# sriramelango/optimized-diffusion-model

Hardware: AMD Instinct MI355X
Metric: trajectories/sec (1000-step PC sampler, NCSN++ [1,9,9], bs=128/GPU) (higher is better)
Workload: dtype f32; 1 GPU; NCSN++ nf=64 ch_mult=[1,2,2] on [128,1,9,9] per GPU, 1000-step reflected PC sampler (predictor euler_maruyama, corrector none), classifier-free guidance on (2B-sample forwards), fp32; global_batch=128, num_scales=1000, score_evals_per_traj=999, parallelism=single GPU

## Files before the change

### optimized-diffusion-model_amd/csrc/common.h

```cpp
#pragma once
#include <hip/hip_runtime.h>

typedef float f32x4 __attribute__((vector_size(16)));

extern __shared__ __attribute__((aligned(16))) unsigned char rdmi_lds[];

#define RDMI_THREADS 256

#if defined(__HIP_DEVICE_COMPILE__)
#define RDMI_SCHED_FENCE() __builtin_amdgcn_sched_barrier(0)
#else
#define RDMI_SCHED_FENCE() ((void)0)
#endif

__device__ __forceinline__ float silu_f(float y) { return __fdividef(y, 1.0f + __expf(-y)); }

__device__ __forceinline__ f32x4 mfma16(float a, float b, f32x4 c) {
    return __builtin_amdgcn_mfma_f32_16x16x4f32(a, b, c, 0, 0, 0);
}

__device__ __forceinline__ f32x4 mfma4(float a, float b, f32x4 c) {
    return __builtin_amdgcn_mfma_f32_4x4x1f32(a, b, c, 0, 0, 0);
}

typedef unsigned short bf16_t;
typedef unsigned int u32x4 __attribute__((vector_size(16)));
#if defined(__HIP_DEVICE_COMPILE__)
typedef __bf16 rdmi_bf16x8 __attribute__((ext_vector_type(8)));
__device__ __forceinline__ bf16_t f2bf(float f) { return __builtin_bit_cast(unsigned short, (__bf16)f); }
__device__ __forceinline__ f32x4 mfma16_bf16(u32x4 a, u32x4 b, f32x4 c) {
    return __builtin_amdgcn_mfma_f32_16x16x32_bf16(__builtin_bit_cast(rdmi_bf16x8, a), __builtin_bit_cast(rdmi_bf16x8, b), c, 0, 0, 0);
}
#else
__device__ __forceinline__ bf16_t f2bf(float f) {
    unsigned u = __builtin_bit_cast(unsigned, f);
    if ((u & 0x7fffffffu) > 0x7f800000u) return (bf16_t)((u >> 16) | 0x40);
    return (bf16_t)((u + 0x7fffu + ((u >> 16) & 1u)) >> 16);
}
#if defined(RDMI_EMU)
__device__ __forceinline__ float bf2f_host(bf16_t h) { const unsigned u = (unsigned)h << 16; return __builtin_bit_cast(float, u); }
__device__ __forceinline__ f32x4 mfma16_bf16(u32x4 a, u32x4 b, f32x4 c) {
    bf16_t A[64][8], B[64][8];
    std::memcpy(A, emu::wave_exchange(&a, 16), sizeof A);
    std::memcpy(B, emu::wave_exchange(&b, 16), sizeof B);
    const int lane = emu::lane_id(), col = lane & 15;
    for (int e = 0; e < 4; ++e) {
        const int r = (lane >> 4) * 4 + e;
        float s = c[e];
        for (int k = 0; k < 32; ++k) s += bf2f_host(A[r + 16 * (k >> 3)][k & 7]) * bf2f_host(B[col + 16 * (k >> 3)][k & 7]);
        c[e] = s;
    }
    return c;
}
#else
__device__ __forceinline__ f32x4 mfma16_bf16(u32x4, u32x4, f32x4 c) { abort(); return c; }
#endif
#endif
#if defined(__HIP_DEVICE_COMPILE__)
__device__ __forceinline__ void wave_order_point() { __builtin_amdgcn_wave_barrier(); }
#elif defined(RDMI_EMU)
__device__ __forceinline__ void wave_order_point() { int z = 0; (void)emu::wave_exchange(&z, sizeof z); }
#else
__device__ __forceinline__ void wave_order_point() {}
#endif
#if defined(__HIP_DEVICE_COMPILE__)
// ... 12 lines not shown
#elif defined(RDMI_EMU)
__device__ __forceinline__ void glds16(const void* g, unsigned wave_off) { std::memcpy(rdmi_lds + wave_off + 16 * emu::lane_id(), g, 16); }
#else
__device__ __forceinline__ void glds16(const void*, unsigned) {}
#endif
#if defined(__HIP_DEVICE_COMPILE__)
__device__ __forceinline__ int mad_u24(int a, int b, int c) { return (int)(__umul24((unsigned)a, (unsigned)b) + (unsigned)c); }
#else
__device__ __forceinline__ int mad_u24(int a, int b, int c) { return a * b + c; }
#endif
__device__ __forceinline__ unsigned pack_bf16x2(float lo, float hi) { return (unsigned)f2bf(lo) | ((unsigned)f2bf(hi) << 16); }
__device__ __forceinline__ float bf2f(bf16_t h) { return __builtin_bit_cast(float, (unsigned)h << 16); }
__device__ __forceinline__ f32x4 ldact4(const float* base, size_t idx, int bf) {
    if (bf) {
        typedef unsigned int u32x2 __attribute__((vector_size(8)));
        const u32x2 u = *reinterpret_cast<const u32x2*>(reinterpret_cast<const bf16_t*>(base) + idx);
        return f32x4{__builtin_bit_cast(float, u[0] << 16), __builtin_bit_cast(float, u[0] & 0xffff0000u), __builtin_bit_cast(float, u[1] << 16),
                     __builtin_bit_cast(float, u[1] & 0xffff0000u)};
    }
    return *reinterpret_cast<const f32x4*>(base + idx);
}
__device__ __forceinline__ float ldact1(const float* base, size_t idx, int bf) { return bf ? bf2f(reinterpret_cast<const bf16_t*>(base)[idx]) : base[idx]; }
__device__ __forceinline__ void stact1(float* base, size_t idx, float v, int bf) {
    if (bf) reinterpret_cast<bf16_t*>(base)[idx] = f2bf(v); else base[idx] = v;
}

#if defined(__HIP_DEVICE_COMPILE__)
template <int CTRL>
__device__ __forceinline__ float dpp_f(float v) {
    return __builtin_bit_cast(float, __builtin_amdgcn_update_dpp(0, __builtin_bit_cast(int, v), CTRL, 0xf, 0xf, true));
}
__device__ __forceinline__ float row16_sum(float v) {
    v += dpp_f<0xB1>(v); v += dpp_f<0x4E>(v); v += dpp_f<0x141>(v); v += dpp_f<0x140>(v);
    return v;
}
__device__ __forceinline__ float row16_max(float v) {
    v = fmaxf(v, dpp_f<0xB1>(v)); v = fmaxf(v, dpp_f<0x4E>(v)); v = fmaxf(v, dpp_f<0x141>(v)); v = fmaxf(v, dpp_f<0x140>(v));
    return v;
}
__device__ __forceinline__ float row8_sum(float v) {
    v += dpp_f<0xB1>(v); v += dpp_f<0x4E>(v); v += dpp_f<0x141>(v);
    return v;
}
__device__ __forceinline__ float lane_bcast(float v, int l) { return __builtin_bit_cast(float, __builtin_amdgcn_readlane(__builtin_bit_cast(int, v), l)); }
#else
__device__ __forceinline__ float row16_sum(float v) { v += __shfl_xor(v, 1); v += __shfl_xor(v, 2); v += __shfl_xor(v, 4); v += __shfl_xor(v, 8); return v; }
__device__ __forceinline__ float row16_max(float v) {
    v = fmaxf(v, __shfl_xor(v, 1)); v = fmaxf(v, __shfl_xor(v, 2)); v = fmaxf(v, __shfl_xor(v, 4)); v = fmaxf(v, __shfl_xor(v, 8));
    return v;
}
__device__ __forceinline__ float row8_sum(float v) { v += __shfl_xor(v, 1); v += __shfl_xor(v, 2); v += __shfl_xor(v, 4); return v; }
__device__ __forceinline__ float lane_bcast(float v, int l) { return __shfl(v, l); }
#endif
__device__ __forceinline__ float group32_sum(float v, int lane) {
    const float r = row16_sum(v);
    const float s0 = lane_bcast(r, 0), s1 = lane_bcast(r, 16), s2 = lane_bcast(r, 32), s3 = lane_bcast(r, 48);
    return lane < 32 ? s0 + s1 : s2 + s3;
}
__device__ __forceinline__ float group64_sum(float v) {
    const float r = row16_sum(v);
    return (lane_bcast(r, 0) + lane_bcast(r, 16)) + (lane_bcast(r, 32) + lane_bcast(r, 48));
}

__device__ __forceinline__ float reflect_f(float x) {
    float m = x - 2.0f * floorf(x * 0.5f);
    m = (m >= 2.0f) ? 0.0f : m;
    return (m > 1.0f) ? 2.0f - m : m;
}

__device__ __forceinline__ f32x4 ldg4(const float* p) {
#if defined(__HIP_DEVICE_COMPILE__)
    typedef const f32x4 __attribute__((address_space(1))) * gptr_t;
    return *(gptr_t)(p);
#else
    return *reinterpret_cast<const f32x4*>(p);
#endif
}
__device__ __forceinline__ float ldg1(const float* p) {
#if defined(__HIP_DEVICE_COMPILE__)
    typedef const float __attribute__((address_space(1))) * gptr_t;
    return *(gptr_t)(p);
#else
    return *p;
#endif
}

__device__ __forceinline__ void stg1(float* p, float v) {
#if defined(__HIP_DEVICE_COMPILE__)
    typedef float __attribute__((address_space(1))) * gptr_t;
    *(gptr_t)(p) = v;
#else
    *p = v;
#endif
}
__device__ __forceinline__ void stg4(float* p, f32x4 v) {
#if defined(__HIP_DEVICE_COMPILE__)
    typedef f32x4 __attribute__((address_space(1))) * gptr_t;
    *(gptr_t)(p) = v;
#else
    *reinterpret_cast<f32x4*>(p) = v;
#endif
}

#if defined(__HIP_DEVICE_COMPILE__)
typedef unsigned int xq_t __attribute__((ext_vector_type(4)));
struct XBuf { __amdgpu_buffer_rsrc_t r; };
// ... 60 lines not shown
```

### optimized-diffusion-model_amd/csrc/rdmi.hip

```cpp
#include <hip/hip_runtime.h>

#include <algorithm>
#include <cmath>
#include <cstdarg>
#include <cstdio>
#include <cstdlib>
#include <cstring>
#include <climits>
#include <map>
#include <memory>
#include <stdexcept>
#include <string>
#include <vector>

#include "../../include/rdmi.h"
#include "attn_kernel.h"
#include "conv_kernel.h"
#include "misc_kernels.h"
#include "unet_kernel.h"
#include "bwd_kernels.h"
#include "opt_kernels.h"
#include "ode_kernels.h"
#include "tiled_kernels.h"

// ... 1337 lines not shown
        o.main_ph.lds_off = in.off; o.main_ph.rs = in.rs; o.main_ph.nch = in.C / 16;
        for (int t = 0; t < 4; ++t) o.tab_off[t] = up4_table(in.H, in.W, t);
        o.w_tile_stride = 4 * in.C * o.Cout_pad * (int)sizeof(float);
        o.dst_off = dst->off; o.dst_rs = dst->rs;
        if (o.main_ph.nch % 8 != 0 || o.rows <= 4 || o.dst_kind != 0 || in.C != Cout || in.hw() != 16 || in.pm || cur_samp < 0 || dst->C != Cout || dst->hw() != o.rows)
            fail_("folded upsample conv: unsupported shape (" + std::to_string(in.H) + "x" + std::to_string(in.W) + " source, " + std::to_string(in.C) + " -> " + std::to_string(Cout) + " channels)");
        dst->pm = true;
        const int idx = emit(o);
        patch_arena(idx, F_W, c->wmap.at(wkey + ".up4"));
        patch_param(idx, F_BIAS, bias_param);
        return idx;
    }
};

FusedBuilder::LT fused_resblock(FusedBuilder& b, const std::string& name, FusedBuilder::LT& xin, int cout, int dense_off) {
    using LT = FusedBuilder::LT;
    const int H = xin.H, W = xin.W;
    const float rs2 = (float)(1.0 / std::sqrt(2.0));
    if (xin.C != cout) {
        LT out = b.talloc(cout, H, W);
        b.conv(xin, H, W, H, W, 1, 0, 1, name + ".NIN_0", 0, cout, name + ".NIN_0.b", 0, 0, &out, 1.f, -1, nullptr, nullptr, "", "");
        b.gn(xin, name + ".GroupNorm_0", true);
        LT h1 = b.talloc(cout, H, W);
        b.conv(xin, H, W, H, W, 1, 1, 9, name + ".Conv_0", 0, cout, name + ".Conv_0.bias", 0, 0, &h1, 1.f, dense_off, nullptr, nullptr, "", "");
        b.tfree(xin);
        b.gn(h1, name + ".GroupNorm_1", true);
        b.conv(h1, H, W, H, W, 1, 1, 9, name + ".Conv_1", 0, cout, name + ".Conv_1.bias", 0, 0, &out, rs2, -1, &out, nullptr, "", "");
        b.tfree(h1);
        return out;
    }
    LT xact = b.talloc(xin.C, H, W);
    b.gn(xact, name + ".GroupNorm_0", true, &xin);
    LT h1 = b.talloc(cout, H, W);
    b.conv(xact, H, W, H, W, 1, 1, 9, name + ".Conv_0", 0, cout, name + ".Conv_0.bias", 0, 0, &h1, 1.f, dense_off, nullptr, nullptr, "", "");
    b.tfree(xact);
    b.gn(h1, name + ".GroupNorm_1", true);
    LT out = b.talloc(cout, H, W);
    b.conv(h1, H, W, H, W, 1, 1, 9, name + ".Conv_1", 0, cout, name + ".Conv_1.bias", 0, 0, &out, rs2, -1, &xin, nullptr, "", "");
    b.tfree(h1);
    b.tfree(xin);
    return out;
}

FusedBuilder::LT fused_attn(FusedBuilder& b, const std::string& name, FusedBuilder::LT& x) {
    using LT = FusedBuilder::LT;
    rdmi_ctx* c = b.c;
    const int C = x.C, H = x.H, W = x.W, L = H * W, Lpad = pad16(L);
    if (C != 64 || Lpad > 96) { b.fail_("attention: only C=64, H*W<=96 is built"); return x; }
    if (b.cur_samp < 0) { b.fail_("attention inside the multi-sample (low-resolution) section is not built"); return x; }
    LT xn = b.talloc(C, H, W);
    b.gn(xn, name + ".GroupNorm_0", false, &x);
    LT q = b.talloc(C, H, W), k = b.talloc(C, H, W);
    const int ps = Lpad + 4;
    const int vt_bytes = C * ps * 4, p_bytes = L * ps * 4;
    const int vt_off = b.alloc_top(vt_bytes);
    const bool fold3 = !b.train && std::getenv("RDMI_NO_ATTN_FOLD") == nullptr;
    const size_t bq = c->wmap.at(name + (fold3 ? ".bqkvf" : ".bqkv"));
    {
        const int idx = b.conv(xn, H, W, H, W, 1, 0, 1, name + (fold3 ? ".qkv3f" : ".qkv3"), 0, 3 * C, "", bq, 3, &q, 1.f, -1, nullptr, nullptr, "", "");
        FOp& o = b.prog.fprog[(size_t)idx];
        o.dst2_off = k.off; o.dst3_off = vt_off; o.dst3_rs = ps; o.split_C = C;
        o.qkv1 = (std::getenv("RDMI_NO_QKV1") == nullptr && o.ntap == 1 && o.main_ph.nch == 4 && o.Cout_pad == 192 && C == 64 && o.mtiles <= 6) ? 1 : 0;
    }
    b.tfree(xn);
    const int p_off = b.alloc_top(p_bytes);
    LT o = b.talloc(C, H, W);
    {
        FOp a = b.blank(FOP_ATTN);
        a.q_off = q.off; a.k_off = k.off; a.qk_rs = q.rs; a.vt_off = vt_off; a.p_off = p_off; a.ps = ps;
        a.L = L; a.Lpad = Lpad; a.C = C; a.att_scale = 1.0f / std::sqrt((float)C);
        a.dst_off = o.off; a.dst_rs = o.rs;
        if (fold3) { a.resid_off = x.off; a.resid_rs = x.rs; a.scale = (float)(1.0 / std::sqrt(2.0)); }
        const int ia = b.emit(a);
        if (fold3) b.patch_param(ia, FusedBuilder::F_BIAS, name + ".NIN_3.b");
    }
    b.tfree(q); b.tfree(k);
    b.free_bytes(vt_off, vt_bytes); b.free_bytes(p_off, p_bytes);
    if (fold3) { b.tfree(x); return o; }
    LT out = b.talloc(C, H, W);
    b.conv(o, H, W, H, W, 1, 0, 1, name + ".NIN_3", 0, C, name + ".NIN_3.b", 0, 0, &out, (float)(1.0 / std::sqrt(2.0)), -1, &x, nullptr, "", "");
    b.tfree(o);
    b.tfree(x);
    return out;
}

int build_fused_program_pass(rdmi_ctx* c, rdmi_ctx::FusedProg& q, int S, int TAB_RESERVE, int TAB1_RESERVE, int* tab_used, int* tab1_used, bool coop, bool train);

int build_one_program(rdmi_ctx* c, int S, bool coop = false, bool train = false) {
    int used = 0, used1 = 0;
    {
        rdmi_ctx::FusedProg sizing;
        if (int e = build_fused_program_pass(c, sizing, S, 8 * 1024, 24 * 1024, &used, &used1, coop, train)) return e;
    }
    rdmi_ctx::FusedProg q;
    if (int e = build_fused_program_pass(c, q, S, (used + 63) & ~63, (used1 + 63) & ~63, &used, &used1, coop, train)) return e;
    c->progs.push_back(std::move(q));
    return 0;
}

int resident_workgroups() {
#ifdef RDMI_EMU
    return 256;
#else
    int dev = 0, cus = 0;
    if (hipGetDevice(&dev) != hipSuccess || hipDeviceGetAttribute(&cus, hipDeviceAttributeMultiprocessorCount, dev) != hipSuccess) return 0;
    return cus;
#endif
// ... 1317 lines not shown
```

### optimized-diffusion-model_amd/csrc/unet_kernel.h

```cpp
#pragma once
#include <cstddef>

#include "common.h"

#define UW_THREADS 512
#define UW_WAVES 8
#ifndef UW_PF_M4
#define UW_PF_M4 4
#endif
#ifndef UW_PF_N1
#define UW_PF_N1 4
#endif
#ifndef UW_PF_KS1
#define UW_PF_KS1 4
#endif
#ifndef UW_PRIO
#define UW_PRIO 0
#endif
#ifndef UW_LIGHT_BARRIER
#define UW_LIGHT_BARRIER 0
#endif

__device__ __forceinline__ void lds_barrier() {
#if defined(__HIP_DEVICE_COMPILE__) && UW_LIGHT_BARRIER
// ... 735 lines not shown
    const int col = nt * 16 + lrow;
    const int gcol = min(col, o_Cout - 1) >> 2, G4 = o_Cout >> 2;
    const float* slots = lds_f(OPI(w, gn_slot_off));
    const float inv_cnt = OPF(w, inv_cnt), eps = OPF(w, eps);
    const int act = OPI(w, gn_act), rs = OPI(w, gn_rs);
    float* dstp = lds_f(OPI(w, gn_off));
    float mean = 0.f, rstd = 0.f;
    if (o_samp >= 0) {
        const float* slot = slots + (size_t)gcol * nslots * 2;
        float s1 = 0.f, s2 = 0.f;
        for (int k = 0; k < nslots; k += 2) {
            const f32x4 p = *reinterpret_cast<const f32x4*>(slot + 2 * k);
            s1 += p[0]; s2 += p[1]; s1 += p[2]; s2 += p[3];
        }
        mean = s1 * inv_cnt;
        rstd = (1.0f / sqrtf(fmaxf(s2 * inv_cnt - mean * mean, 0.f) + eps)) * gmul;
    }
#pragma unroll
    for (int i = 0; i < 4; ++i)
        if (i < nmt) {
            if (o_samp < 0) {
                float s1, s2;
                if (hw_shift == 4) {
                    const float* slot = slots + (size_t)((mt0 + i * WM) * G4 + gcol) * 8;
                    const f32x4 p = *reinterpret_cast<const f32x4*>(slot), q = *reinterpret_cast<const f32x4*>(slot + 4);
                    s1 = (p[0] + p[2]) + (q[0] + q[2]); s2 = (p[1] + p[3]) + (q[1] + q[3]);
                } else { s1 = ps1[i]; s2 = ps2[i]; }
                mean = s1 * inv_cnt;
                rstd = (1.0f / sqrtf(fmaxf(s2 * inv_cnt - mean * mean, 0.f) + eps)) * gmul;
            }
            const int row0 = (mt0 + i * WM) * 16 + kq * 4;
#pragma unroll
            for (int r = 0; r < 4; ++r) {
                const float y = (acc[i][r] - mean) * rstd + gadd;
                float ya = act ? silu_f(y) : y;
                if (TR) {
                    const int dop = OPI(w, drop_op);
                    if (dop >= 0 && u.drop_p > 0.f)
                        ya *= dropout_scale((uint64_t)*u.seed_dev, (uint32_t)dop, ((uint64_t)min(n0, u.NB - 1) * o_rows + (row0 + r)) * o_Cout + col, u.drop_p);
                }
                if (row0 + r < o_rows && col < o_Cout) dstp[(row0 + r) * rs + col] = ya;
            }
        }
}

__device__ __forceinline__ void fconv_qkv(const OpW& w, const UnetArgs& u, int wave, int lane) {
    const int lrow = lane & 15, kq = lane >> 4;
    const int wn = wave & 3, wm = wave >> 2;
    const int o_rows = OPI(w, rows), mtiles = OPI(w, mtiles), o_Cout_pad = OPI(w, Cout_pad);
    const int m_lds = OPI(w, main_ph.lds_off), m_rs = OPI(w, main_ph.rs);
    const float* m_w = OPP(w, const float, main_ph.w);
    const float* o_bias = OPP(w, const float, bias);
    const float o_scale = OPF(w, scale);
    const int sc_ = OPI(w, split_C), o_dst = OPI(w, dst_off), o_dst2 = OPI(w, dst2_off), o_dst3 = OPI(w, dst3_off), o_dst_rs = OPI(w, dst_rs), rs3 = OPI(w, dst3_rs);
    const short* tab = reinterpret_cast<const short*>(rdmi_lds + opw_at(w, (int)(offsetof(FOp, tab_off) / 4)));
    const size_t bstride = (size_t)o_Cout_pad * 16;
    f32x4 bf[3][4];
    float add[3];
#pragma unroll
    for (int c = 0; c < 3; ++c) {
        const int col = (wn + 4 * c) * 16 + lrow;
        add[c] = ldg1(o_bias + col);
#pragma unroll
        for (int ch = 0; ch < 4; ++ch) bf[c][ch] = ldg4(m_w + (size_t)col * 16 + kq * 4 + (size_t)ch * bstride);
    }
    int abase[3];
#pragma unroll
    for (int i = 0; i < 3; ++i) abase[i] = arow(tab, min((wm + 2 * i) * 16 + lrow, mtiles * 16 - 1), m_lds, m_rs, u.zero_off) + kq * 16;
    f32x4 acc[3][3];
#pragma unroll
    for (int i = 0; i < 3; ++i)
#pragma unroll
        for (int c = 0; c < 3; ++c) acc[i][c] = f32x4{0.f, 0.f, 0.f, 0.f};
#pragma unroll
    for (int ch = 0; ch < 4; ++ch) {
        f32x4 af[3];
#pragma unroll
        for (int i = 0; i < 3; ++i) af[i] = *reinterpret_cast<const f32x4*>(rdmi_lds + abase[i] + ch * 64);
#pragma unroll
        for (int j = 0; j < 4; ++j)
#pragma unroll
            for (int i = 0; i < 3; ++i)
#pragma unroll
                for (int c = 0; c < 3; ++c) acc[i][c] = mfma16(af[i][j], bf[c][ch][j], acc[i][c]);
    }
    const int lc = wn * 16 + lrow;
    (void)sc_;
#pragma unroll
    for (int i = 0; i < 3; ++i) {
        const int mt = wm + 2 * i;
        if (mt >= mtiles) continue;
        const int row0 = mt * 16 + kq * 4;
#pragma unroll
        for (int c = 0; c < 2; ++c) {
            float* dstp = lds_f(c == 0 ? o_dst : o_dst2);
#pragma unroll
            for (int r = 0; r < 4; ++r)
                if (row0 + r < o_rows) dstp[(row0 + r) * o_dst_rs + lc] = (acc[i][c][r] + add[c]) * o_scale;
        }
        f32x4 v = acc[i][2];
        for (int r = 0; r < 4; ++r) v[r] = (v[r] + add[2]) * o_scale;
        *reinterpret_cast<f32x4*>(lds_f(o_dst3) + lc * rs3 + row0) = v;
    }
}

template <bool DIAG, bool MS, bool TR = false>
__device__ __forceinline__ void fop_conv(const OpW& w, const UnetArgs& u, int n0, int wave, int lane, long long* fine) {
    const int ntiles = OPI(w, Cout_pad) >> 4, mtiles = OPI(w, mtiles);
    const int lWN = (ntiles >= 8 && (ntiles & 7) == 0) ? 3 : (ntiles >= 4 ? 2 : (ntiles >= 2 ? 1 : 0));
    const int WN = 1 << lWN, WM = UW_WAVES >> lWN, lWM = 3 - lWN;
    const int wn = wave & (WN - 1), wm = wave >> lWN;
    const int o_Cout = OPI(w, Cout), o_dense = OPI(w, dense_off);
    const float* o_bias = OPP(w, const float, bias); const float* o_bias2 = OPP(w, const float, bias2);
    if (OPI(w, dst_kind) == 3 && OPI(w, qkv1)) { fconv_qkv(w, u, wave, lane); return; }
    const bool fused_gn = OPI(w, dst_kind) == 0 && OPI(w, gn_off) >= 0;
    const int wts = OPI(w, w_tile_stride);
    const int o_samp = MS ? OPI(w, samp) : 0, hw_shift = MS ? OPI(w, hw_shift) : 0;
    const float* dense_base = u.dense + (size_t)max(o_dense, 0);
    f32x4 acc[4];
    float ps1[4] = {0.f, 0.f, 0.f, 0.f}, ps2[4] = {0.f, 0.f, 0.f, 0.f};
    const int wcol = min(wn * 16 + (lane & 15), o_Cout - 1);
    float gmul = ldg1((fused_gn ? OPP(w, const float, gamma) : o_bias) + wcol), gadd = ldg1((fused_gn ? OPP(w, const float, beta) : o_bias) + wcol);
    int k_mt0 = 0, k_nt = 0, k_nmt = 0;
    for (int nt = wn; nt < ntiles; nt += WN) {
        const int col = nt * 16 + (lane & 15), colc = min(col, o_Cout - 1);
        float add1 = ldg1(o_bias + colc), add2 = ldg1((o_bias2 ? o_bias2 : o_bias) + colc);
        for (int mt0 = wm; mt0 < mtiles; mt0 += wts ? WM : 4 * WM) {
            const int left = (mtiles - mt0 + WM - 1) >> lWM;
            const int nmt = wts ? 1 : (left >= 4 ? 4 : left);
            float daddm[4] = {0.f, 0.f, 0.f, 0.f};
            float dv = ldg1(dense_base + (o_dense >= 0 ? (size_t)min(n0 + max(o_samp, 0), u.NB - 1) * u.dense_stride + colc : 0));
            if (MS && o_dense >= 0 && o_samp < 0) {
#pragma unroll
                for (int i = 0; i < 4; ++i)
                    if (i < nmt) {
                        const int sl = ((mt0 + i * WM) * 16 + (lane >> 4) * 4) >> hw_shift;
                        daddm[i] = ldg1(dense_base + (size_t)min(n0 + sl, u.NB - 1) * u.dense_stride + colc);
                    }
            }
            const bool tapm = (OPI(w, main_ph.nch) & 3) == 0;
            const bool tapm8 = (OPI(w, main_ph.nch) & 7) == 0;
            switch (nmt) {
                case 1:
                    if (OPI(w, rows) <= 4 && OPI(w, dst_kind) != 1 && OPI(w, dst_kind) != 3) {
                        if (tapm8) fconv_main_t<DIAG, 1, false, 8, true>(w, u, mt0, WM, nt, lane, fine, acc);
                        else fconv_main<DIAG, 1, UW_PF_M4, true>(w, u, mt0, WM, nt, lane, fine, acc);
                    } else if (tapm8) fconv_main_t<DIAG, 1, false, 8>(w, u, mt0, WM, nt, lane, fine, acc, (unsigned)mt0 * (unsigned)wts);
                    else if (tapm) fconv_main_t<DIAG, 1>(w, u, mt0, WM, nt, lane, fine, acc);
                    else fconv_main<DIAG, 1, UW_PF_N1>(w, u, mt0, WM, nt, lane, fine, acc);
                    break;
                case 2: fconv_main<DIAG, 2, 8>(w, u, mt0, WM, nt, lane, fine, acc); break;
                case 3: {
                    const int last_rows = OPI(w, rows) - (mt0 + 2 * WM) * 16;
                    const bool lm4 = last_rows >= 1 && last_rows <= 4 && OPI(w, dst_kind) != 1 && OPI(w, dst_kind) != 3;
                    if (tapm) { if (lm4) fconv_main_t<DIAG, 3, true>(w, u, mt0, WM, nt, lane, fine, acc); else fconv_main_t<DIAG, 3>(w, u, mt0, WM, nt, lane, fine, acc); }
// ... 114 lines not shown
#pragma unroll
    for (int k = 0; k < KMAX; ++k) {
        const int p = tid + k * UW_THREADS;
        if (p < np && !withhold) {
            f32x2 v;
            if (mode == 0) v = *reinterpret_cast<const f32x2*>(lds_f(0) + at(p, m));
            else {
                const int i = p << 1, row = i >> csh, c = i & (Cs - 1);
                v = *reinterpret_cast<const f32x2*>(lds_f(a_off) + row * a_rs + c);
                *reinterpret_cast<f32x2*>(lds_f(0) + at(p, m)) = v;
            }
            const float v0 = v[0], v1 = v[1];
            xbuf_store16(xb, gbase + (unsigned)m * slotb + (unsigned)p * 16u, __builtin_bit_cast(unsigned, v0), __builtin_bit_cast(unsigned, v1), epoch);
        }
    }
    const int nk = (np + UW_THREADS - 1) / UW_THREADS;
    u32x4 y[3 * KMAX];
    unsigned long long spins = 0;
    bool broken = __hip_atomic_load(u.coop_err, __ATOMIC_RELAXED, __HIP_MEMORY_SCOPE_AGENT) != 0;
    if (broken) *failw = 1;
    for (; !broken;) {
#pragma unroll
        for (int k = 0; k < KMAX; ++k)
            if (k < nk) {
                const unsigned po = (unsigned)min(tid + k * UW_THREADS, np - 1) * 16u;
#pragma unroll
                for (int jj = 0; jj < 3; ++jj) y[k * 3 + jj] = xbuf_load16(xb, gbase + (unsigned)((m + 1 + jj) & 3) * slotb + po);
            }
        bool ok = true;
#pragma unroll
        for (int k = 0; k < KMAX; ++k)
            if (k < nk) {
#pragma unroll
                for (int jj = 0; jj < 3; ++jj) { const unsigned t1 = y[k * 3 + jj][1], t3 = y[k * 3 + jj][3]; ok &= t1 == epoch && t3 == epoch; }
            }
        if (ok) break;
        if (++spins > RDMI_SPIN_LIMIT) { *failw = 1; __hip_atomic_store(u.coop_err, 1, __ATOMIC_RELAXED, __HIP_MEMORY_SCOPE_AGENT); break; }
        spin_relax();
    }
#pragma unroll
    for (int k = 0; k < KMAX; ++k) {
        const int p = tid + k * UW_THREADS;
        if (!broken && k < nk && p < np) {
#pragma unroll
            for (int jj = 0; jj < 3; ++jj) {
                const unsigned a = y[k * 3 + jj][0], b = y[k * 3 + jj][2];
                *reinterpret_cast<f32x2*>(lds_f(0) + at(p, (m + 1 + jj) & 3)) = f32x2{__builtin_bit_cast(float, a), __builtin_bit_cast(float, b)};
            }
        }
    }
}

__device__ __forceinline__ void fop_attn(const OpW& w, int wave, int lane) {
    struct { int L, Lpad, q_off, k_off, vt_off, p_off, qk_rs, ps, C, dst_off, dst_rs; float att_scale; } o;
    o.L = OPI(w, L); o.Lpad = OPI(w, Lpad); o.q_off = OPI(w, q_off); o.k_off = OPI(w, k_off); o.vt_off = OPI(w, vt_off); o.p_off = OPI(w, p_off);
    o.qk_rs = OPI(w, qk_rs); o.ps = OPI(w, ps); o.C = OPI(w, C); o.dst_off = OPI(w, dst_off); o.dst_rs = OPI(w, dst_rs); o.att_scale = OPF(w, att_scale);
    const int lrow = lane & 15, kq = lane >> 4;
    const int L = o.L, mtiles = o.Lpad >> 4;
    const float* Q = lds_f(o.q_off);
    const float* K = lds_f(o.k_off);
    const float* Vt = lds_f(o.vt_off);
    float* P = lds_f(o.p_off);
    const int rs = o.qk_rs, ps = o.ps;
    const int nchq = o.C >> 4;
    for (int mt = wave; mt < mtiles; mt += UW_WAVES) {
        f32x4 s[6];
#pragma unroll
        for (int t = 0; t < 6; ++t) s[t] = f32x4{0.f, 0.f, 0.f, 0.f};
        const int qrow = min(mt * 16 + lrow, L - 1);
        for (int ch = 0; ch < nchq; ++ch) {
            const f32x4 af = *reinterpret_cast<const f32x4*>(Q + (size_t)qrow * rs + ch * 16 + kq * 4);
#pragma unroll
            for (int t = 0; t < 6; ++t) {
                if (t < mtiles) {
                    const int krow = min(t * 16 + lrow, L - 1);
                    const f32x4 bf = *reinterpret_cast<const f32x4*>(K + (size_t)krow * rs + ch * 16 + kq * 4);
#pragma unroll
                    for (int j = 0; j < 4; ++j) s[t] = mfma16(af[j], bf[j], s[t]);
                }
            }
        }
#pragma unroll
        for (int r = 0; r < 4; ++r) {
            float mx = -3.0e38f;
#pragma unroll
            for (int t = 0; t < 6; ++t)
                if (t < mtiles && t * 16 + lrow < L) { s[t][r] *= o.att_scale; mx = fmaxf(mx, s[t][r]); }
            mx = row16_max(mx);
            float sum = 0.f;
#pragma unroll
            for (int t = 0; t < 6; ++t)
                if (t < mtiles) {
                    const float e = (t * 16 + lrow < L) ? __expf(s[t][r] - mx) : 0.f;
                    s[t][r] = e;
                    sum += e;
                }
            sum = row16_sum(sum);
            const float inv = 1.0f / sum;
            const int row = mt * 16 + kq * 4 + r;
            if (row < L) {
#pragma unroll
                for (int t = 0; t < 6; ++t)
                    if (t < mtiles) P[(size_t)row * ps + t * 16 + lrow] = s[t][r] * inv;
            }
        }
    }
    lds_barrier();
    {
        const int wn = wave & 3, wm = wave >> 2;
        const int col = wn * 16 + lrow;
        f32x4 acc[3];
#pragma unroll
        for (int i = 0; i < 3; ++i) acc[i] = f32x4{0.f, 0.f, 0.f, 0.f};
        for (int ch = 0; ch < mtiles; ++ch) {
            const f32x4 bf = *reinterpret_cast<const f32x4*>(Vt + (size_t)col * ps + ch * 16 + kq * 4);
#pragma unroll
            for (int i = 0; i < 3; ++i) {
                const int mt = wm + 2 * i;
                if (mt < mtiles) {
                    const int prow = min(mt * 16 + lrow, L - 1);
                    const f32x4 af = *reinterpret_cast<const f32x4*>(P + (size_t)prow * ps + ch * 16 + kq * 4);
#pragma unroll
                    for (int j = 0; j < 4; ++j) acc[i] = mfma16(af[j], bf[j], acc[i]);
                }
            }
        }
        float* O = lds_f(o.dst_off);
        const float* b3 = OPP(w, const float, bias);
        const int o_resid = OPI(w, resid_off), o_resid_rs = OPI(w, resid_rs);
        const float o_scale = OPF(w, scale), badd = b3 ? ldg1(b3 + col) : 0.f;
#pragma unroll
        for (int i = 0; i < 3; ++i) {
            const int mt = wm + 2 * i;
            if (mt < mtiles)
                for (int r = 0; r < 4; ++r) {
                    const int row = mt * 16 + kq * 4 + r;
                    if (row < L) {
                        float v = acc[i][r];
                        if (b3) v = (v + badd + lds_f(o_resid)[(size_t)row * o_resid_rs + col]) * o_scale;
                        O[(size_t)row * o.dst_rs + col] = v;
                    }
                }
        }
    }
}

template <bool DIAG, bool MS = false, bool COOP = false, bool TRAIN = false>
__global__ __launch_bounds__(UW_THREADS) void unet_wg_kernel(UnetArgs u) {
    const int tid = threadIdx.x, lane = tid & 63;
    const int wave = __builtin_amdgcn_readfirstlane(tid >> 6);
    int n = MS ? blockIdx.x * u.S : blockIdx.x, n_multi = n, n_spill = n, spill_cap = u.NB;
    int cg = 0, cm = 0;
    if (COOP) {
        const int st = u.coop_stride, bid = blockIdx.x, blk = bid / (4 * st), r = bid - blk * 4 * st;
        cm = r / st; cg = blk * st + (r - cm * st);
        if (cg * 4 >= u.NB) return;
        n = min(cg * 4 + cm, u.NB - 1);
        n_multi = cg * 4;
        n_spill = bid * 4; spill_cap = 0x7fffffff;
    }
    {
        const int nw = u.tab_bytes >> 2;
        const int* src = reinterpret_cast<const int*>(u.tabs);
        int* dst = reinterpret_cast<int*>(rdmi_lds + u.tab_base);
        for (int i = tid; i < nw; i += UW_THREADS) dst[i] = src[i];
        float* z = lds_f(u.zero_off);
        for (int i = tid; i < (u.zero_bytes >> 2); i += UW_THREADS) z[i] = 0.f;
    }
#if defined(__HIP_DEVICE_COMPILE__) && UW_PRIO == 1
    if (wave >= 4) __builtin_amdgcn_s_setprio(1);
#elif defined(__HIP_DEVICE_COMPILE__) && UW_PRIO == 2
    if (wave < 4) __builtin_amdgcn_s_setprio(1);
#endif
    float* stat = lds_f(u.zero_off + u.zero_bytes);
    int* const failw = reinterpret_cast<int*>(stat) + 270;
    if (COOP && tid == 0) *failw = 0;
    if (DIAG && u.stamps && n == 0 && tid == 0) u.stamps[0] = clock64();
    OpW cur = opw_load(u.prog, lane);
    OpW nxt = opw_load(u.prog + (u.nops > 1 ? 1 : 0), lane);
    f32x4 pgm = {1.f, 1.f, 1.f, 1.f}, pbt = {0.f, 0.f, 0.f, 0.f};
    gn_prefetch(cur, tid, pgm, pbt);
    for (int pc = 0; pc < u.nops; ++pc) {
        const OpW nn = opw_load(u.prog + (pc + 2 < u.nops ? pc + 2 : u.nops - 1), lane);
        long long* fine = (DIAG && u.stamps && n == 0 && tid == ((u.dbg >> 16) & 7) * 64) ? u.stamps + 1024 + pc * 8 : nullptr;
        const int kind = OPI(cur, kind);
        if (DIAG && fine) fine[2] = clock64();
        f32x4 ngm = pgm, nbt = pbt;
        if (pc + 1 < u.nops) gn_prefetch(nxt, tid, ngm, nbt);
        if (DIAG && fine) fine[3] = clock64();
        const int skip = (DIAG && u.dbg) ? ((kind == FOP_GN ? 4 : kind == FOP_CONV ? 8 : kind == FOP_ATTN ? 16 : 32) & u.dbg) : 0;
        const bool multi = MS && OPI(cur, samp) < 0;
        switch (skip ? -1 : kind) {
            case FOP_GATHER: fop_gather<MS>(cur, u, multi ? n_spill : n, multi ? spill_cap : u.NB, COOP ? cm : 0, tid); break;
            case FOP_STORE: fop_store<MS>(cur, u, multi ? n_spill : n, multi ? spill_cap : u.NB, tid); break;
            case FOP_GN: fop_gn<MS>(cur, stat, tid, pgm, pbt, DIAG ? u.dbg : 0); break;
// ... 26 lines not shown
```

Measured before the change: 183.2 trajectories/s.

## Restructure attention as split-K flash-style softmax with edge-row handling

Attention is rewritten so each wave computes S^T tiles for one query tile over half the key tiles, does an online softmax, and multiplies by V in registers, storing partial max/sum/output. A final pass merges the two halves, which removes the full P matrix write to LDS and the second barrier-separated GEMM. When L mod 16 == 1 (e.g. 81 = 5*16+1), the single leftover row or column is handled with scalar FMA and cross-row reductions instead of a wasted 16-row MFMA tile. The QKV projection applies the same trick and skips its third MFMA tile when no wave owns it. The cost is more complex code, an extra merge step, and reliance on permlane swap intrinsics.

```diff
diff --git a/optimized-diffusion-model_amd/csrc/common.h b/optimized-diffusion-model_amd/csrc/common.h
--- a/optimized-diffusion-model_amd/csrc/common.h
+++ b/optimized-diffusion-model_amd/csrc/common.h
@@ -11,6 +11,12 @@
 #define RDMI_SCHED_FENCE() __builtin_amdgcn_sched_barrier(0)
 #else
 #define RDMI_SCHED_FENCE() ((void)0)
+#endif
+
+#if defined(__HIP_DEVICE_COMPILE__)
+__device__ __forceinline__ float rcp_f(float x) { return __builtin_amdgcn_rcpf(x); }
+#else
+__device__ __forceinline__ float rcp_f(float x) { return 1.0f / x; }
 #endif
 
 __device__ __forceinline__ float silu_f(float y) { return __fdividef(y, 1.0f + __expf(-y)); }
@@ -129,6 +135,27 @@
 __device__ __forceinline__ float row8_sum(float v) { v += __shfl_xor(v, 1); v += __shfl_xor(v, 2); v += __shfl_xor(v, 4); return v; }
 __device__ __forceinline__ float lane_bcast(float v, int l) { return __shfl(v, l); }
 #endif
+#if defined(__HIP_DEVICE_COMPILE__)
+__device__ __forceinline__ float xrow_sum(float v) {
+    unsigned x = __builtin_bit_cast(unsigned, v);
+    const auto a = __builtin_amdgcn_permlane16_swap(x, x, false, false);
+    v = __builtin_bit_cast(float, (unsigned)a[0]) + __builtin_bit_cast(float, (unsigned)a[1]);
+    x = __builtin_bit_cast(unsigned, v);
+    const auto b = __builtin_amdgcn_permlane32_swap(x, x, false, false);
+    return __builtin_bit_cast(float, (unsigned)b[0]) + __builtin_bit_cast(float, (unsigned)b[1]);
+}
+__device__ __forceinline__ float xrow_max(float v) {
+    unsigned x = __builtin_bit_cast(unsigned, v);
+    const auto a = __builtin_amdgcn_permlane16_swap(x, x, false, false);
+    v = fmaxf(__builtin_bit_cast(float, (unsigned)a[0]), __builtin_bit_cast(float, (unsigned)a[1]));
+    x = __builtin_bit_cast(unsigned, v);
+    const auto b = __builtin_amdgcn_permlane32_swap(x, x, false, false);
+    return fmaxf(__builtin_bit_cast(float, (unsigned)b[0]), __builtin_bit_cast(float, (unsigned)b[1]));
+}
+#else
+__device__ __forceinline__ float xrow_sum(float v) { v += __shfl_xor(v, 16); v += __shfl_xor(v, 32); return v; }
+__device__ __forceinline__ float xrow_max(float v) { v = fmaxf(v, __shfl_xor(v, 16)); v = fmaxf(v, __shfl_xor(v, 32)); return v; }
+#endif
 __device__ __forceinline__ float group32_sum(float v, int lane) {
     const float r = row16_sum(v);
     const float s0 = lane_bcast(r, 0), s1 = lane_bcast(r, 16), s2 = lane_bcast(r, 32), s3 = lane_bcast(r, 48);
diff --git a/optimized-diffusion-model_amd/csrc/rdmi.hip b/optimized-diffusion-model_amd/csrc/rdmi.hip
--- a/optimized-diffusion-model_amd/csrc/rdmi.hip
+++ b/optimized-diffusion-model_amd/csrc/rdmi.hip
@@ -1413,7 +1413,8 @@
     b.gn(xn, name + ".GroupNorm_0", false, &x);
     LT q = b.talloc(C, H, W), k = b.talloc(C, H, W);
     const int ps = Lpad + 4;
-    const int vt_bytes = C * ps * 4, p_bytes = L * ps * 4;
+    const int nt_mfma = (L & 15) == 1 ? L / 16 : Lpad / 16;
+    const int vt_bytes = C * ps * 4, p_bytes = (384 + nt_mfma * 1024 + 128) * 4;
     const int vt_off = b.alloc_top(vt_bytes);
     const bool fold3 = !b.train && std::getenv("RDMI_NO_ATTN_FOLD") == nullptr;
     const size_t bq = c->wmap.at(name + (fold3 ? ".bqkvf" : ".bqkv"));
diff --git a/optimized-diffusion-model_amd/csrc/unet_kernel.h b/optimized-diffusion-model_amd/csrc/unet_kernel.h
--- a/optimized-diffusion-model_amd/csrc/unet_kernel.h
+++ b/optimized-diffusion-model_amd/csrc/unet_kernel.h
@@ -811,9 +811,11 @@
     const float* m_w = OPP(w, const float, main_ph.w);
     const float* o_bias = OPP(w, const float, bias);
     const float o_scale = OPF(w, scale);
-    const int sc_ = OPI(w, split_C), o_dst = OPI(w, dst_off), o_dst2 = OPI(w, dst2_off), o_dst3 = OPI(w, dst3_off), o_dst_rs = OPI(w, dst_rs), rs3 = OPI(w, dst3_rs);
+    const int o_dst = OPI(w, dst_off), o_dst2 = OPI(w, dst2_off), o_dst3 = OPI(w, dst3_off), o_dst_rs = OPI(w, dst_rs), rs3 = OPI(w, dst3_rs);
     const short* tab = reinterpret_cast<const short*>(rdmi_lds + opw_at(w, (int)(offsetof(FOp, tab_off) / 4)));
     const size_t bstride = (size_t)o_Cout_pad * 16;
+    const bool edge = (o_rows & 15) == 1;
+    const int nmt = edge ? mtiles - 1 : mtiles;
     f32x4 bf[3][4];
     float add[3];
 #pragma unroll
@@ -826,6 +828,7 @@
     int abase[3];
 #pragma unroll
     for (int i = 0; i < 3; ++i) abase[i] = arow(tab, min((wm + 2 * i) * 16 + lrow, mtiles * 16 - 1), m_lds, m_rs, u.zero_off) + kq * 16;
+    const bool three = wm + 4 < nmt;
     f32x4 acc[3][3];
 #pragma unroll
     for (int i = 0; i < 3; ++i)
@@ -839,16 +842,21 @@
 #pragma unroll
         for (int j = 0; j < 4; ++j)
 #pragma unroll
-            for (int i = 0; i < 3; ++i)
+            for (int i = 0; i < 2; ++i)
 #pragma unroll
                 for (int c = 0; c < 3; ++c) acc[i][c] = mfma16(af[i][j], bf[c][ch][j], acc[i][c]);
+        if (three) {
+#pragma unroll
+            for (int j = 0; j < 4; ++j)
+#pragma unroll
+                for (int c = 0; c < 3; ++c) acc[2][c] = mfma16(af[2][j], bf[c][ch][j], acc[2][c]);
+        }
     }
     const int lc = wn * 16 + lrow;
-    (void)sc_;
 #pragma unroll
     for (int i = 0; i < 3; ++i) {
         const int mt = wm + 2 * i;
-        if (mt >= mtiles) continue;
+        if (mt >= nmt) continue;
         const int row0 = mt * 16 + kq * 4;
 #pragma unroll
         for (int c = 0; c < 2; ++c) {
@@ -860,6 +868,26 @@
         f32x4 v = acc[i][2];
         for (int r = 0; r < 4; ++r) v[r] = (v[r] + add[2]) * o_scale;
         *reinterpret_cast<f32x4*>(lds_f(o_dst3) + lc * rs3 + row0) = v;
+    }
+    if (edge && wm == 1) {
+        const int er = o_rows - 1;
+        const float* a = reinterpret_cast<const float*>(rdmi_lds + arow(tab, er, m_lds, m_rs, u.zero_off)) + kq * 4;
+        float d[3] = {0.f, 0.f, 0.f};
+#pragma unroll
+        for (int ch = 0; ch < 4; ++ch) {
+            const f32x4 x = *reinterpret_cast<const f32x4*>(a + ch * 16);
+#pragma unroll
+            for (int j = 0; j < 4; ++j)
+#pragma unroll
+                for (int c = 0; c < 3; ++c) d[c] = fmaf(x[j], bf[c][ch][j], d[c]);
+        }
+#pragma unroll
+        for (int c = 0; c < 3; ++c) d[c] = (xrow_sum(d[c]) + add[c]) * o_scale;
+        if (kq == 0) {
+            lds_f(o_dst)[er * o_dst_rs + lc] = d[0];
+            lds_f(o_dst2)[er * o_dst_rs + lc] = d[1];
+            *reinterpret_cast<f32x4*>(lds_f(o_dst3) + lc * rs3 + er) = f32x4{d[2], 0.f, 0.f, 0.f};
+        }
     }
 }
 
@@ -1080,95 +1108,177 @@
 }
 
 __device__ __forceinline__ void fop_attn(const OpW& w, int wave, int lane) {
-    struct { int L, Lpad, q_off, k_off, vt_off, p_off, qk_rs, ps, C, dst_off, dst_rs; float att_scale; } o;
-    o.L = OPI(w, L); o.Lpad = OPI(w, Lpad); o.q_off = OPI(w, q_off); o.k_off = OPI(w, k_off); o.vt_off = OPI(w, vt_off); o.p_off = OPI(w, p_off);
-    o.qk_rs = OPI(w, qk_rs); o.ps = OPI(w, ps); o.C = OPI(w, C); o.dst_off = OPI(w, dst_off); o.dst_rs = OPI(w, dst_rs); o.att_scale = OPF(w, att_scale);
+    const int L = OPI(w, L), rs = OPI(w, qk_rs), ps = OPI(w, ps), dst_rs = OPI(w, dst_rs);
+    const float att_scale = OPF(w, att_scale);
     const int lrow = lane & 15, kq = lane >> 4;
-    const int L = o.L, mtiles = o.Lpad >> 4;
-    const float* Q = lds_f(o.q_off);
-    const float* K = lds_f(o.k_off);
-    const float* Vt = lds_f(o.vt_off);
-    float* P = lds_f(o.p_off);
-    const int rs = o.qk_rs, ps = o.ps;
-    const int nchq = o.C >> 4;
-    for (int mt = wave; mt < mtiles; mt += UW_WAVES) {
-        f32x4 s[6];
-#pragma unroll
-        for (int t = 0; t < 6; ++t) s[t] = f32x4{0.f, 0.f, 0.f, 0.f};
-        const int qrow = min(mt * 16 + lrow, L - 1);
-        for (int ch = 0; ch < nchq; ++ch) {
-            const f32x4 af = *reinterpret_cast<const f32x4*>(Q + (size_t)qrow * rs + ch * 16 + kq * 4);
-#pragma unroll
-            for (int t = 0; t < 6; ++t) {
-                if (t < mtiles) {
-                    const int krow = min(t * 16 + lrow, L - 1);
-                    const f32x4 bf = *reinterpret_cast<const f32x4*>(K + (size_t)krow * rs + ch * 16 + kq * 4);
-#pragma unroll
-                    for (int j = 0; j < 4; ++j) s[t] = mfma16(af[j], bf[j], s[t]);
-                }
-            }
-        }
+    const float* Q = lds_f(OPI(w, q_off));
+    const float* K = lds_f(OPI(w, k_off));
+    const float* Vt = lds_f(OPI(w, vt_off));
+    float* st = lds_f(OPI(w, p_off));
+    float* O = lds_f(OPI(w, dst_off));
+    const float* b3 = OPP(w, const float, bias);
+    const float* resid = lds_f(max(OPI(w, resid_off), 0));
+    const int resid_rs = OPI(w, resid_rs);
+    const float o_scale = OPF(w, scale);
+    const bool edge = (L & 15) == 1;
+    const int nt = edge ? (L >> 4) : ((L + 15) >> 4);
+    const int kA = (nt + 1) >> 1;
+    const bool hasB = nt > kA || (edge && nt > 0);
+    const int nunits = hasB ? 2 * nt : nt;
+    float* part = st + 384;
+    float* pe_row = part + nt * 1024;
+    f32x4 acc[4];
+#pragma unroll 1
+    for (int it = 0; it < 2; ++it) {
+        const int idx = it ? wave : 15 - wave;
+        if (idx >= nunits) continue;
+        const int g = idx >= nt ? 1 : 0, m = g ? idx - nt : idx;
+        const int t0 = g ? kA : 0, ntl = g ? nt - kA : kA;
+        const bool ek = g && edge;
+        const int qrow = min(m * 16 + lrow, L - 1);
+        f32x4 s[3];
+#pragma unroll
+        for (int i = 0; i < 3; ++i) s[i] = f32x4{0.f, 0.f, 0.f, 0.f};
+        float se = 0.f, mx = -3.0e38f;
+        const int klim = L - kq * 4;
+#pragma unroll 1
+        for (int ch = 0; ch < 4; ++ch) {
+            const f32x4 qf = *reinterpret_cast<const f32x4*>(Q + qrow * rs + ch * 16 + kq * 4);
+#pragma unroll
+            for (int i = 0; i < 3; ++i)
+                if (i < ntl) {
+                    const int krow = min((t0 + i) * 16 + lrow, L - 1);
+                    const f32x4 kf = *reinterpret_cast<const f32x4*>(K + krow * rs + ch * 16 + kq * 4);
+#pragma unroll
+                    for (int j = 0; j < 4; ++j) s[i] = mfma16(kf[j], qf[j], s[i]);
+                }
+            if (ek) {
+                const f32x4 kf = *reinterpret_cast<const f32x4*>(K + (L - 1) * rs + ch * 16 + kq * 4);
+#pragma unroll
+                for (int j = 0; j < 4; ++j) se = fmaf(qf[j], kf[j], se);
+            }
+        }
+        if (ek) { se = xrow_sum(se) * att_scale; mx = se; }
+#pragma unroll
+        for (int i = 0; i < 3; ++i)
+            if (i < ntl) {
+#pragma unroll
+                for (int r = 0; r < 4; ++r) {
+                    s[i][r] = ((t0 + i) * 16 + r < klim) ? s[i][r] * att_scale : -3.0e38f;
+                    mx = fmaxf(mx, s[i][r]);
+                }
+            }
+        mx = xrow_max(mx);
+        float sum = 0.f;
+#pragma unroll
+        for (int i = 0; i < 3; ++i)
+            if (i < ntl) {
+#pragma unroll
+                for (int r = 0; r < 4; ++r) {
+                    s[i][r] = __expf(s[i][r] - mx);
+                    sum += s[i][r];
+                }
+            }
+        sum = xrow_sum(sum);
+#pragma unroll
+        for (int c = 0; c < 4; ++c) acc[c] = f32x4{0.f, 0.f, 0.f, 0.f};
+#pragma unroll
+        for (int i = 0; i < 3; ++i)
+            if (i < ntl) {
+                f32x4 vf[4];
+#pragma unroll
+                for (int c = 0; c < 4; ++c) vf[c] = *reinterpret_cast<const f32x4*>(Vt + (c * 16 + lrow) * ps + (t0 + i) * 16 + kq * 4);
+#pragma unroll
+                for (int j = 0; j < 4; ++j)
+#pragma unroll
+                    for (int c = 0; c < 4; ++c) acc[c] = mfma16(s[i][j], vf[c][j], acc[c]);
+            }
+        if (ek) {
+            const float pe = __expf(se - mx);
+            sum += pe;
+#pragma unroll
+            for (int c = 0; c < 4; ++c) {
+                acc[c] = mfma16(kq == 0 ? pe : 0.f, Vt[(c * 16 + lrow) * ps + L - 1], acc[c]);
+            }
+        }
+        if (kq == 0) {
+            st[(g * 6 + m) * 32 + lrow] = mx; st[(g * 6 + m) * 32 + 16 + lrow] = sum;
+            if (!hasB) { st[(6 + m) * 32 + lrow] = -3.0e38f; st[(6 + m) * 32 + 16 + lrow] = 0.f; }
+        }
+        if (g || !hasB) {
+#pragma unroll
+            for (int c = 0; c < 4; ++c) *reinterpret_cast<f32x4*>(part + ((m * 4 + c) * 64 + lane) * 4) = acc[c];
+        }
+    }
+    if (edge && wave == 5) {
+        const float* qe = Q + (L - 1) * rs;
+        const int k0 = min(lane, L - 1), k1 = min(64 + lane, L - 1);
+        float s0 = 0.f, s1 = 0.f;
+#pragma unroll 2
+        for (int i = 0; i < 16; ++i) {
+            const f32x4 qv = *reinterpret_cast<const f32x4*>(qe + i * 4);
+            const f32x4 a = *reinterpret_cast<const f32x4*>(K + k0 * rs + i * 4), b = *reinterpret_cast<const f32x4*>(K + k1 * rs + i * 4);
+#pragma unroll
+            for (int j = 0; j < 4; ++j) { s0 = fmaf(qv[j], a[j], s0); s1 = fmaf(qv[j], b[j], s1); }
+        }
+        s0 *= att_scale; s1 *= att_scale;
+        const bool v0 = lane < L, v1 = 64 + lane < L;
+        float mx = -3.0e38f;
+        if (v0) mx = s0;
+        if (v1) mx = fmaxf(mx, s1);
+        mx = row16_max(mx);
+        mx = fmaxf(fmaxf(lane_bcast(mx, 0), lane_bcast(mx, 16)), fmaxf(lane_bcast(mx, 32), lane_bcast(mx, 48)));
+        const float e0 = v0 ? __expf(s0 - mx) : 0.f, e1 = v1 ? __expf(s1 - mx) : 0.f;
+        const float inv = rcp_f(group64_sum(e0 + e1));
+        pe_row[lane] = e0 * inv; pe_row[64 + lane] = e1 * inv;
+        wave_order_point();
+        float o = 0.f;
+#pragma unroll 1
+        for (int t = 0; t < nt; ++t)
+#pragma unroll
+            for (int k4 = 0; k4 < 4; ++k4) {
+                const f32x4 p = *reinterpret_cast<const f32x4*>(pe_row + t * 16 + k4 * 4), v = *reinterpret_cast<const f32x4*>(Vt + lane * ps + t * 16 + k4 * 4);
+#pragma unroll
+                for (int j = 0; j < 4; ++j) o = fmaf(p[j], v[j], o);
+            }
+        o = fmaf(pe_row[L - 1], Vt[lane * ps + L - 1], o);
+        if (b3) o = (o + ldg1(b3 + lane) + resid[(L - 1) * resid_rs + lane]) * o_scale;
+        O[(L - 1) * dst_rs + lane] = o;
+    }
+    lds_barrier();
+    if (wave < nt) {
+        const int m = wave;
+        const f32x4 ma = *reinterpret_cast<const f32x4*>(st + m * 32 + kq * 4), sa = *reinterpret_cast<const f32x4*>(st + m * 32 + 16 + kq * 4);
+        const f32x4 mb = *reinterpret_cast<const f32x4*>(st + (6 + m) * 32 + kq * 4), sb = *reinterpret_cast<const f32x4*>(st + (6 + m) * 32 + 16 + kq * 4);
+        f32x4 wa, wb;
 #pragma unroll
         for (int r = 0; r < 4; ++r) {
-            float mx = -3.0e38f;
-#pragma unroll
-            for (int t = 0; t < 6; ++t)
-                if (t < mtiles && t * 16 + lrow < L) { s[t][r] *= o.att_scale; mx = fmaxf(mx, s[t][r]); }
-            mx = row16_max(mx);
-            float sum = 0.f;
-#pragma unroll
-            for (int t = 0; t < 6; ++t)
-                if (t < mtiles) {
-                    const float e = (t * 16 + lrow < L) ? __expf(s[t][r] - mx) : 0.f;
-                    s[t][r] = e;
-                    sum += e;
-                }
-            sum = row16_sum(sum);
-            const float inv = 1.0f / sum;
-            const int row = mt * 16 + kq * 4 + r;
+            const float mm = fmaxf(ma[r], mb[r]), fa = __expf(ma[r] - mm), fb = __expf(mb[r] - mm);
+            const float inv = rcp_f(sa[r] * fa + sb[r] * fb);
+            wa[r] = fa * inv; wb[r] = fb * inv;
+        }
+        const bool has3 = b3 != nullptr;
+        const float sc = o_scale;
+        f32x4 ob[4];
+        float badd[4] = {0.f, 0.f, 0.f, 0.f};
+#pragma unroll
+        for (int c = 0; c < 4; ++c) ob[c] = *reinterpret_cast<const f32x4*>(part + ((m * 4 + c) * 64 + lane) * 4);
+        if (has3) {
+#pragma unroll
+            for (int c = 0; c < 4; ++c) badd[c] = ldg1(b3 + c * 16 + lrow);
+        }
+#pragma unroll
+        for (int r = 0; r < 4; ++r) {
+            const int row = m * 16 + kq * 4 + r;
             if (row < L) {
-#pragma unroll
-                for (int t = 0; t < 6; ++t)
-                    if (t < mtiles) P[(size_t)row * ps + t * 16 + lrow] = s[t][r] * inv;
-            }
-        }
-    }
-    lds_barrier();
-    {
-        const int wn = wave & 3, wm = wave >> 2;
-        const int col = wn * 16 + lrow;
-        f32x4 acc[3];
-#pragma unroll
-        for (int i = 0; i < 3; ++i) acc[i] = f32x4{0.f, 0.f, 0.f, 0.f};
-        for (int ch = 0; ch < mtiles; ++ch) {
-            const f32x4 bf = *reinterpret_cast<const f32x4*>(Vt + (size_t)col * ps + ch * 16 + kq * 4);
-#pragma unroll
-            for (int i = 0; i < 3; ++i) {
-                const int mt = wm + 2 * i;
-                if (mt < mtiles) {
-                    const int prow = min(mt * 16 + lrow, L - 1);
-                    const f32x4 af = *reinterpret_cast<const f32x4*>(P + (size_t)prow * ps + ch * 16 + kq * 4);
-#pragma unroll
-                    for (int j = 0; j < 4; ++j) acc[i] = mfma16(af[j], bf[j], acc[i]);
-                }
-            }
-        }
-        float* O = lds_f(o.dst_off);
-        const float* b3 = OPP(w, const float, bias);
-        const int o_resid = OPI(w, resid_off), o_resid_rs = OPI(w, resid_rs);
-        const float o_scale = OPF(w, scale), badd = b3 ? ldg1(b3 + col) : 0.f;
-#pragma unroll
-        for (int i = 0; i < 3; ++i) {
-            const int mt = wm + 2 * i;
-            if (mt < mtiles)
-                for (int r = 0; r < 4; ++r) {
-                    const int row = mt * 16 + kq * 4 + r;
-                    if (row < L) {
-                        float v = acc[i][r];
-                        if (b3) v = (v + badd + lds_f(o_resid)[(size_t)row * o_resid_rs + col]) * o_scale;
-                        O[(size_t)row * o.dst_rs + col] = v;
-                    }
-                }
+                const float* rp = resid + row * resid_rs + lrow;
+                float* op = O + row * dst_rs + lrow;
+#pragma unroll
+                for (int c = 0; c < 4; ++c) {
+                    const float v = acc[c][r] * wa[r] + ob[c][r] * wb[r], x = rp[c * 16];
+                    op[c * 16] = (v + badd[c] + (has3 ? x : 0.f)) * sc;
+                }
+            }
         }
     }
 }
```

New measurement: 184.9 trajectories/s, median of 6. No clear change (+0.9%).
